# yifita/iso-points

Hardware: AMD Instinct MI355X
Metric: Mpoints/s full iso-point cycle (project+resample+splat), 1M pts (higher is better)
Workload: dtype f32-class (split-fp16 operands, 2^-22: hidden-layer products from two fp16 parts per f32 operand under exact power-of-two scales, 3 fp16-MFMA passes, f32 accumulate; everything else f32)

## Files before the change

### include/isopoints.h

```cpp
#ifndef ISOPOINTS_H_
#define ISOPOINTS_H_

#include <stdint.h>

#ifdef __cplusplus
extern "C" {
#endif

#define ISO_OK 0
#define ISO_ERR_INVALID (-1)
#define ISO_ERR_UNSUPPORTED (-2)
#define ISO_ERR_LAUNCH (-3)
#define ISO_ERR_WORKSPACE (-4)

const char* iso_version(void);
const char* iso_last_error(void);


int iso_project_sphere(const float* pts_in, float* pts_out, float* normals_out,
                       uint8_t* mask_out, int64_t n, float cx, float cy,
                       float cz, float radius, int max_iters, float tol,
                       void* stream);

typedef struct iso_follow {
  void* grid_ws; int64_t grid_n_max;
  const float* views; int n_views; float znear; float zfar; int backface_culling;
  int32_t* mask_out; void* front_ws; int64_t front_ws_bytes;
  int64_t* first_idx_out; int64_t* num_pts_out; int32_t* view_total_out;
} iso_follow;

int iso_project_sphere_follow(const float* pts_in, float* pts_out, float* normals_out,
                              uint8_t* mask_out, int64_t n, float cx, float cy,
                              float cz, float radius, int max_iters, float tol,
                              const iso_follow* follow_host, void* stream);

int64_t iso_siren_raw_floats(int hidden, int n_hidden);
int64_t iso_siren_packed_floats(int hidden, int n_hidden);
int iso_siren_pack_weights(const float* raw, float* packed, int hidden,
                           int n_hidden, void* stream);
int iso_siren_set_gemm_mode(int mode);
int iso_siren_get_gemm_mode(void);
int iso_siren_set_tail_from(int first_tail_iteration);
int iso_siren_set_drawn_tiles(int on);
int iso_idr_set_drawn_tiles(int on);
int iso_siren_set_step_form(int form);
int iso_siren_get_step_form(void);
int iso_siren_step_form_used(int hidden, int n_hidden, int coded);
int iso_siren_step_kernel(int hidden, int n_hidden, int value_only, int coded);
int iso_siren_step_launches(int hidden, int n_hidden, int max_iters);
int64_t iso_project_siren_workspace_bytes(int64_t n, int hidden, int n_hidden);
int64_t iso_project_siren_counts_offset(int64_t n, int hidden, int n_hidden);
int iso_project_siren(const float* pts_in, float* pts_out, float* normals_out,
                      uint8_t* mask_out, int64_t n, const float* packed,
                      int hidden, int n_hidden, float omega_first,
                      float omega_hidden, int max_iters, float tol,
                      void* workspace, int64_t workspace_bytes, void* stream);
int iso_siren_sdf_grad(const float* pts, float* sdf_out, float* grad_out,
                       int64_t n, const float* packed, int hidden,
                       int n_hidden, float omega_first, float omega_hidden,
                       void* workspace, int64_t workspace_bytes, void* stream);

int iso_siren_fold_codes(const float* w0c, const float* b0, const float* codes, float* table, int hidden,
                         int padded_hidden, int c_dim, int64_t n_codes, void* stream);
int iso_project_siren_coded(const float* pts_in, float* pts_out, float* normals_out,
                            uint8_t* mask_out, int64_t n, const float* packed,
                            int hidden, int n_hidden, float omega_first,
                            float omega_hidden, int max_iters, float tol,
                            void* workspace, int64_t workspace_bytes, void* stream,
                            const float* code_bias, const int32_t* code_of, int64_t n_codes);
int iso_siren_sdf_grad_coded(const float* pts, float* sdf_out, float* grad_out,
                             int64_t n, const float* packed, int hidden,
                             int n_hidden, float omega_first, float omega_hidden,
                             void* workspace, int64_t workspace_bytes, void* stream,
                             const float* code_bias, const int32_t* code_of, int64_t n_codes);

int iso_idr_set_gemm_mode(int mode);
int iso_idr_get_gemm_mode(void);
int iso_idr_step_form(int hidden, int n_layers, int skip_layer, int n_freq, int value_only);
int64_t iso_idr_raw_floats(int hidden, int n_layers, int skip_layer, int n_freq);
int64_t iso_idr_packed_floats(int hidden, int n_layers);
int iso_idr_pack_weights(const float* raw, float* packed, int hidden, int n_layers,
                         int skip_layer, int n_freq, void* stream);
int64_t iso_project_idr_workspace_bytes(int64_t n, int hidden, int n_layers);
int iso_project_idr(const float* pts_in, float* pts_out, float* normals_out, uint8_t* mask_out,
                    int64_t n, const float* packed, int hidden, int n_layers, int skip_layer,
                    int n_freq, float beta, int max_iters, float tol, void* workspace,
                    int64_t workspace_bytes, void* stream);
int iso_idr_sdf_grad(const float* pts, float* sdf_out, float* grad_out, int64_t n,
                     const float* packed, int hidden, int n_layers, int skip_layer, int n_freq,
                     float beta, void* workspace, int64_t workspace_bytes, void* stream);

int iso_trace_sphere(const float* ray0, const float* dirs, float* pts_out, float* sdf_out,
// ... 428 lines not shown
```

### iso_points_amd/_lib.py

```python
import ctypes
import os

import torch

_HERE = os.path.dirname(os.path.abspath(__file__))
LIB_PATH = os.path.join(_HERE, "libisopoints_hip.so")
if os.environ.get("ISO_DEV_LIB"):
    LIB_PATH = os.path.abspath(os.environ["ISO_DEV_LIB"])

_c = ctypes
_P = _c.c_void_p
_I = _c.c_int
_L = _c.c_int64
_F = _c.c_float

SIGNATURES = {
    "iso_version": (_c.c_char_p, []),
    "iso_last_error": (_c.c_char_p, []),
    "iso_project_sphere": (_I, [_P, _P, _P, _P, _L, _F, _F, _F, _F, _I, _F, _P]),
    "iso_project_sphere_follow": (_I, [_P, _P, _P, _P, _L, _F, _F, _F, _F, _I, _F, _P, _P]),
    "iso_siren_raw_floats": (_L, [_I, _I]),
    "iso_siren_packed_floats": (_L, [_I, _I]),
    "iso_siren_set_gemm_mode": (_I, [_I]),
    "iso_siren_get_gemm_mode": (_I, []),
    "iso_siren_set_tail_from": (_I, [_I]),
    "iso_siren_set_drawn_tiles": (_I, [_I]),
    "iso_idr_set_drawn_tiles": (_I, [_I]),
    "iso_siren_set_step_form": (_I, [_I]),
    "iso_siren_get_step_form": (_I, []),
    "iso_siren_step_form_used": (_I, [_I, _I, _I]),
    "iso_siren_step_kernel": (_I, [_I, _I, _I, _I]),
    "iso_siren_step_launches": (_I, [_I, _I, _I]),
    "iso_siren_pack_weights": (_I, [_P, _P, _I, _I, _P]),
    "iso_project_siren_workspace_bytes": (_L, [_L, _I, _I]),
    "iso_project_siren_counts_offset": (_L, [_L, _I, _I]),
    "iso_project_siren": (_I, [_P, _P, _P, _P, _L, _P, _I, _I, _F, _F, _I, _F, _P, _L, _P]),
    "iso_siren_sdf_grad": (_I, [_P, _P, _P, _L, _P, _I, _I, _F, _F, _P, _L, _P]),
    "iso_idr_set_gemm_mode": (_I, [_I]),
    "iso_idr_get_gemm_mode": (_I, []),
    "iso_idr_step_form": (_I, [_I, _I, _I, _I, _I]),
    "iso_idr_raw_floats": (_L, [_I, _I, _I, _I]),
    "iso_idr_packed_floats": (_L, [_I, _I]),
    "iso_idr_pack_weights": (_I, [_P, _P, _I, _I, _I, _I, _P]),
    "iso_project_idr_workspace_bytes": (_L, [_L, _I, _I]),
    "iso_project_idr": (_I, [_P, _P, _P, _P, _L, _P, _I, _I, _I, _I, _F, _I, _F, _P, _L, _P]),
    "iso_idr_sdf_grad": (_I, [_P, _P, _P, _L, _P, _I, _I, _I, _I, _F, _P, _L, _P]),
    "iso_trace_sphere": (_I, [_P, _P, _P, _P, _P, _L, _F, _F, _F, _F, _F, _F, _I, _F, _P]),
    "iso_trace_siren": (_I, [_P, _P, _P, _P, _P, _L, _P, _I, _I, _F, _F, _F, _F, _I, _F, _P, _L, _P]),
    "iso_siren_fold_codes": (_I, [_P, _P, _P, _P, _I, _I, _I, _L, _P]),
    "iso_project_siren_coded": (_I, [_P, _P, _P, _P, _L, _P, _I, _I, _F, _F, _I, _F, _P, _L, _P, _P, _P, _L]),
    "iso_siren_sdf_grad_coded": (_I, [_P, _P, _P, _L, _P, _I, _I, _F, _F, _P, _L, _P, _P, _P, _L]),
    "iso_trace_siren_coded": (_I, [_P, _P, _P, _P, _P, _L, _P, _I, _I, _F, _F, _F, _F, _I, _F, _P, _L, _P, _P, _P, _L]),
    "iso_trace_idr": (_I, [_P, _P, _P, _P, _P, _L, _P, _I, _I, _I, _I, _F, _F, _F, _I, _F, _P, _L, _P]),
    "iso_ray_nearest_point_workspace_bytes": (_L, [_L]),
    "iso_ray_nearest_point": (_I, [_P, _L, _F, _F, _F, _P, _L, _P, _P, _P, _P, _L, _P]),
    "iso_raymarch_settle": (_I, [_P, _P, _L, _P, _P, _P, _P, _F, _I, _I, _P, _P, _P, _P]),
    "iso_raymarch_overshoot": (_I, [_P, _P, _L, _P, _P, _P, _P, _I, _I, _F, _P, _P, _P, _P]),
    "iso_raymarch_secant": (_I, [_P, _P, _L, _P, _P, _P, _P, _P, _P, _P, _P]),
    "iso_image_sample": (_I, [_P, _I, _I, _I, _I, _P, _L, _I, _P, _P]),
    "iso_ear_candidates": (_I, [_P, _P, _P, _P, _L, _I, _F, _P, _P, _P]),
    "iso_points_bbox": (_I, [_P, _P, _I, _L, _P, _P]),
    "iso_frnn_make_grid": (_I, [_P, _P, _P, _I, _L, _I, _P, _P]),
    "iso_frnn_make_grid_density": (_I, [_P, _P, _P, _I, _L, _I, _F, _P, _P]),
    "iso_frnn_insert_points": (_I, [_P, _P, _P, _P, _P, _P, _I, _L, _L, _I, _P]),
    "iso_prefix_sum_workspace_bytes": (_L, [_L, _I]),
    "iso_prefix_sum": (_I, [_P, _P, _L, _I, _L, _P, _L, _P]),
    "iso_frnn_scan_cells": (_I, [_P, _P, _P, _I, _L, _I, _P, _L, _P]),
    "iso_frnn_counting_sort": (_I, [_P, _P, _P, _P, _P, _P, _P, _I, _L, _L, _I, _P]),
    "iso_frnn_query_workspace_bytes": (_L, [_I, _L, _L]),
    "iso_frnn_query": (_I, [_P, _P, _P, _P, _P, _P, _P, _P, _P, _I, _P, _P, _P, _I, _L, _L, _L, _P, _L, _P]),
    "iso_frnn_query_others": (_I, [_P, _P, _P, _P, _P, _P, _P, _I, _P, _P, _P, _I, _L, _L, _P, _L, _P]),
    "iso_frnn_gather": (_I, [_P, _P, _P, _I, _L, _L, _I, _I, _P]),
    "iso_repulse": (_I, [_P, _P, _P, _L, _P, _L, _L, _I, _P, _P]),
    "iso_upsample_candidates": (_I, [_P, _P, _L, _I, _P, _P, _P]),
    "iso_farthest_point_sampling_work_floats": (_L, [_I, _L]),
    "iso_farthest_point_sampling": (_I, [_P, _P, _P, _P, _I, _L, _L, _P, _P, _P]),
    "iso_farthest_point_sampling_form": (_I, [_L, _I]),
    "iso_pca_frames_work_bytes": (_L, [_I]),
    "iso_pca_frames": (_I, [_P, _P, _P, _I, _L, _I, _I, _P, _P, _P, _P]),
    "iso_pca_frames_backward_work_bytes": (_L, [_I, _L, _I]),
    "iso_pca_frames_backward": (_I, [_P, _P, _P, _I, _L, _I, _I, _P, _P, _P, _P, _P, _L, _P, _P]),
    "iso_splat_view_flags": (_I, [_P, _P, _P, _P, _L, _I, _F, _F, _I, _P]),
    "iso_compact_rows": (_I, [_P, _P, _P, _P, _L, _L, _I, _P]),
    "iso_splat_vrk_h": (_I, [_P, _P, _P, _P, _P, _I, _L, _P]),
    "iso_splat_setup": (_I, [_P, _P, _P, _P, _P, _P, _P, _I, _L, _I, _F, _F, _P, _P, _P, _P, _P, _P]),
    "iso_splat_vrk_h_global_work_bytes": (_L, [_I]),
# ... 149 lines not shown
```

### iso_points_amd/csrc/siren.hip

```cpp
#include <stdlib.h>
#include <string.h>
#include "siren_common.h"

namespace {

bool siren_shape_ok(int H, int L) {
  return (H == 64 || H == 128 || H == 256) && L >= 0 && L <= 8;
}

int g_gemm_mode = -1;
int gemm_mode() {
  if (g_gemm_mode < 0) {
    const char* e = getenv("ISO_SIREN_GEMM");
    g_gemm_mode = (e && (!strcmp(e, "f32") || !strcmp(e, "0"))) ? 0 : 1;
  }
  return g_gemm_mode;
}

int g_step_form = 1;

int siren_form(int hidden, int n_hidden, bool value_only, bool coded) {
  if (!siren_shape_ok(hidden, n_hidden)) return -1;
  const int NT = hidden / 16;
  if (gemm_mode() == 0 || !siren_x3_supported(hidden, n_hidden)) return 100 + NT;
  if (value_only) return 200 + NT;
  if (hidden == 256 && g_step_form == 1 && (n_hidden == 2 || n_hidden == 3) && !coded) return 500 + NT;
  return (hidden == 128 ? 300 : 400) + NT;
}

int siren_launch_form(int form, const SirenCodedArgs& a, int64_t n, hipStream_t s) {
  switch (form / 100) {
    case 1: return siren_f32_launch(a, 16 * (form % 100), n, s);
    case 2: case 3: case 4: case 5: return siren_x3_launch(form, a, n, s);
    default: return -1;
  }
}

bool form_splits(int form) { return form / 100 >= 4; }

int g_tail_from = -1;
int siren_tail_first(int form, int max_iters) {
  if (!form_splits(form) || g_tail_from == 0) return max_iters + 1;
  if (g_tail_from > 0) return g_tail_from;
  return max_iters >= 6 ? 4 : 2;
}

int g_dyn_tiles = -1;

int64_t stash_floats_any(int H, int L) {
  int64_t a = siren_f32_stash_floats(H, L);
  int64_t b = siren_x3_supported(H, L) ? siren_x3_stash_floats(H, L) : 0;
  return a > b ? a : b;
}

constexpr int kTileCtrInts = 128;
struct SirenCarve {
  int64_t idxA, idxB, tail, tail_counts, counts, tile_ctr, end, tail_cap;
};
SirenCarve siren_carve(int64_t n, int H, int L) {
  if (n < 0) n = 0;
  const int64_t blocks = siren_x3_tail_blocks(), tiles = (n + 31) / 32;
  SirenCarve c;
  c.tail_cap = ((tiles + blocks - 1) / blocks + 1) * 32;
  c.idxA = stash_floats_any(H, L) * 4;
  c.idxB = c.idxA + n * 4;
  c.tail = c.idxB + n * 4;
  c.tail_counts = c.tail + blocks * 2 * c.tail_cap * 4;
  c.counts = c.tail_counts + blocks * 2 * 4;
  c.tile_ctr = c.counts + 64 * 4;
  c.end = c.tile_ctr + kTileCtrInts * 4 + 64;
  return c;
}

__global__ void k_siren_zero(int32_t* c, int n, int32_t* tc, int m) {
  const int i = blockIdx.x * blockDim.x + threadIdx.x;
  if (i < n) c[i] = 0;
  if (i < m) tc[i] = 0;
}

struct SirenTrace { const float* dirs; float alpha, bound; };
struct SirenCodes { const float* bias; const int32_t* of; };

int siren_codes_ok(const char* who, const float* code_bias, const int32_t* code_of, int64_t n_codes) {
  ISO_REQUIRE(code_bias && n_codes >= 1 && (code_of || n_codes == 1), ISO_ERR_INVALID,
              "%s: needs a bias table of n_codes >= 1 rows (and code_of when n_codes > 1)", who);
  return ISO_OK;
}

int siren_run(const char* who, bool ptrs_ok, const float* pts_in, float* pts_out, float* normals_out, uint8_t* mask_out,
              float* sdf_out, float* grad_out, int64_t n, const float* packed, int hidden, int n_hidden, float omega_first,
              float omega_hidden, int max_iters, float tol, void* workspace, int64_t workspace_bytes, void* stream,
              bool eval_only, const SirenTrace* trace, SirenCodes codes) {
  ISO_REQUIRE(siren_shape_ok(hidden, n_hidden), ISO_ERR_UNSUPPORTED,
// ... 56 lines not shown
  ISO_CHECK_LAUNCH(who);
  return ISO_OK;
}

}

extern "C" int64_t iso_siren_raw_floats(int hidden, int n_hidden) {
  int64_t H = hidden;
  return H * 3 + H + (int64_t)n_hidden * (H * H + H) + H + 1;
}

extern "C" int64_t iso_siren_packed_floats(int hidden, int n_hidden) {
  return siren_packed_total(hidden, n_hidden);
}

extern "C" int iso_siren_set_gemm_mode(int mode) {
  ISO_REQUIRE(mode == 0 || mode == 1, ISO_ERR_INVALID, "iso_siren_set_gemm_mode: mode must be 0 (f32 MFMA) or 1 (split fp16)");
  g_gemm_mode = mode;
  return ISO_OK;
}
extern "C" int iso_siren_get_gemm_mode(void) { return gemm_mode(); }

extern "C" int iso_siren_set_step_form(int form) {
  ISO_REQUIRE(form == 0 || form == 1, ISO_ERR_INVALID, "iso_siren_set_step_form: 0 (eight waves, global stash) or 1 (four waves, stash on chip)");
  g_step_form = form;
  return ISO_OK;
}
extern "C" int iso_siren_get_step_form(void) { return g_step_form; }

extern "C" int iso_siren_set_drawn_tiles(int on) {
  ISO_REQUIRE(on >= -1 && on <= 1, ISO_ERR_INVALID, "iso_siren_set_drawn_tiles: -1 (default), 0 or 1");
  g_dyn_tiles = on;
  return ISO_OK;
}

extern "C" int iso_siren_set_tail_from(int first_tail_iteration) {
  ISO_REQUIRE(first_tail_iteration >= -1, ISO_ERR_INVALID, "iso_siren_set_tail_from: -1 (default), 0 (never) or an iteration >= 1");
  g_tail_from = first_tail_iteration;
  return ISO_OK;
}

extern "C" int iso_siren_step_kernel(int hidden, int n_hidden, int value_only, int coded) {
  return siren_form(hidden, n_hidden, value_only != 0, coded != 0);
}
extern "C" int iso_siren_step_form_used(int hidden, int n_hidden, int coded) {
  return siren_form(hidden, n_hidden, false, coded != 0) / 100 == 5 ? 1 : 0;
}
extern "C" int iso_siren_step_launches(int hidden, int n_hidden, int max_iters) {
  if (max_iters < 0) return 0;
  const int from = siren_tail_first(siren_form(hidden, n_hidden, false, false), max_iters);
  return from <= max_iters && from > 0 ? from + 1 : max_iters + 1;
}

extern "C" int iso_siren_pack_weights(const float* raw, float* packed, int hidden,
                                      int n_hidden, void* stream) {
  ISO_REQUIRE(siren_shape_ok(hidden, n_hidden), ISO_ERR_UNSUPPORTED,
              "iso_siren_pack_weights: hidden must be 64/128/256 and 0<=n_hidden<=8 (got %d, %d)",
              hidden, n_hidden);
  ISO_REQUIRE(raw && packed, ISO_ERR_INVALID, "iso_siren_pack_weights: null pointer");
  siren_f32_pack(raw, packed, hidden, n_hidden, (hipStream_t)stream);
  if (hidden % 32 == 0) siren_x3_pack(raw, packed, hidden, n_hidden, (hipStream_t)stream);
  ISO_CHECK_LAUNCH("iso_siren_pack_weights");
  return ISO_OK;
}

extern "C" int64_t iso_project_siren_workspace_bytes(int64_t n, int hidden, int n_hidden) {
  return siren_carve(n, hidden, n_hidden).end;
}
extern "C" int64_t iso_project_siren_counts_offset(int64_t n, int hidden, int n_hidden) {
  return siren_carve(n, hidden, n_hidden).counts;
}

__global__ void k_siren_fold_codes(const float* __restrict__ w0c, const float* __restrict__ b0,
                                   const float* __restrict__ codes, float* __restrict__ table, int H, int Hp, int C,
                                   int64_t U) {
  const int64_t total = U * Hp;
  for (int64_t o = (int64_t)blockIdx.x * blockDim.x + threadIdx.x; o < total; o += (int64_t)gridDim.x * blockDim.x) {
    const int64_t u = o / Hp;
    const int f = (int)(o - u * Hp);
    float v = 0.f;
    if (f < H) {
      double acc = (double)b0[f];
      const float* wr = w0c + (int64_t)f * C;
      const float* cu = codes + u * C;
      for (int k = 0; k < C; ++k) acc = fma((double)wr[k], (double)cu[k], acc);
      v = (float)acc;
    }
    table[o] = v;
  }
}

extern "C" int iso_siren_fold_codes(const float* w0c, const float* b0, const float* codes, float* table, int hidden,
                                    int padded_hidden, int c_dim, int64_t n_codes, void* stream) {
  ISO_REQUIRE(hidden >= 1 && padded_hidden >= hidden && c_dim >= 1 && n_codes >= 0, ISO_ERR_INVALID,
              "iso_siren_fold_codes: bad sizes (hidden %d, padded %d, c_dim %d, codes %lld)", hidden, padded_hidden,
              c_dim, (long long)n_codes);
  if (n_codes == 0) return ISO_OK;
  ISO_REQUIRE(w0c && b0 && codes && table, ISO_ERR_INVALID, "iso_siren_fold_codes: null pointer");
  const int64_t total = n_codes * padded_hidden;
  hipLaunchKernelGGL(k_siren_fold_codes, dim3(iso_stream_grid(total, 256)), dim3(256), 0, (hipStream_t)stream, w0c, b0,
                     codes, table, hidden, padded_hidden, c_dim, n_codes);
  ISO_CHECK_LAUNCH("iso_siren_fold_codes");
  return ISO_OK;
}

static int project_siren(const char* who, const float* pts_in, float* pts_out, float* normals_out, uint8_t* mask_out,
                         int64_t n, const float* packed, int hidden, int n_hidden, float omega_first, float omega_hidden,
                         int max_iters, float tol, void* workspace, int64_t workspace_bytes, void* stream, SirenCodes codes) {
  return siren_run(who, pts_in && pts_out && normals_out && mask_out, pts_in, pts_out, normals_out, mask_out, nullptr,
                   nullptr, n, packed, hidden, n_hidden, omega_first, omega_hidden, max_iters, tol, workspace,
                   workspace_bytes, stream, false, nullptr, codes);
}

extern "C" int iso_project_siren(const float* pts_in, float* pts_out, float* normals_out,
// ... 77 lines not shown
```

### iso_points_amd/csrc/siren_common.h

```cpp
#pragma once
#include "iso_common.h"

struct SirenArgs {
  float* pts;
  float* normals;
  uint8_t* mask;
  float* sdf_out;
  float* grad_out;
  const int32_t* idx_in;
  const int32_t* count_in;
  int32_t* idx_out;
  int32_t* count_out;
  const float* packed;
  float* stash;
  int64_t n;
  int L;
  float w0, wh, tol;
  int do_move;
  int eval_only;
  const float* dirs = nullptr;
  float alpha = 1.f, bound = 0.f, tol_valid = 0.f;
  int fwd_only = 0;
  int64_t cnt_lo = -1, cnt_hi = INT64_MAX;
  int small_tiles = 0;
  int split = 0;
  int big_blocks = 0;
  int32_t* tail_lists = nullptr;
  int32_t* tail_counts = nullptr;
  int32_t* iter_counts = nullptr;
  int tail_cap = 0, it_first = 0, it_last = 0;
  int32_t* tile_ctr = nullptr;
  int draw_first = 0;
  int ps_guard = 0;
};

struct SirenCodedArgs : SirenArgs {
  const float* code_bias = nullptr;
  const int32_t* code_of = nullptr;
};
template <bool CODED> struct SirenArgsOf { using type = SirenArgs; };
template <> struct SirenArgsOf<true> { using type = SirenCodedArgs; };

__host__ __device__ inline int64_t siren_split_point(int64_t count) {
  const int64_t big = 256 * 96, small = 256 * 32;
  const int64_t full = count / big * big, rem = count - full;
  if (rem == 0) return count;
  return (rem + small - 1) / small <= 2 ? full : count;
}

__host__ __device__ inline int64_t off_w0(int H) { (void)H; return 0; }
__host__ __device__ inline int64_t off_wl(int H) { return 4 * (int64_t)H; }
__host__ __device__ inline int64_t off_bl(int H) { return 5 * (int64_t)H; }
__host__ __device__ inline int64_t off_hidden(int H, int l) {
  return 5 * (int64_t)H + 4 + (int64_t)l * ((int64_t)H + 2 * (int64_t)H * H);
}

__host__ __device__ inline int x3_feat(int s, int kappa) {
  return 32 * (s >> 1) + 16 * (s & 1) + 8 * ((kappa & 7) >> 2) + 4 * (kappa >> 3) + (kappa & 3);
}
__host__ __device__ inline int64_t x3_base(int H, int L) { return off_hidden(H, L); }
__host__ __device__ inline int64_t x3_off_w0(int H, int L) { return x3_base(H, L); }
__host__ __device__ inline int64_t x3_off_wl(int H, int L) { return x3_base(H, L) + 4 * (int64_t)H; }
__host__ __device__ inline int64_t x3_off_layer(int H, int L, int l) {
  return x3_base(H, L) + 5 * (int64_t)H + (int64_t)l * (int64_t)H;
}
constexpr int kX16Header = 24;
__host__ __device__ inline int64_t x16_base(int H, int L) { return x3_off_layer(H, L, L); }
__host__ __device__ inline int64_t x16_off_layer(int H, int L, int l) { return x16_base(H, L) + kX16Header + (int64_t)l * H * H; }
__host__ __device__ inline int64_t x16_off_bw(int H, int L, int l) { return x16_off_layer(H, L, L) + (int64_t)l * H * H; }
__host__ __device__ inline int64_t siren_packed_total(int H, int L) { return x16_off_bw(H, L, L); }

void siren_f32_pack(const float* raw, float* packed, int H, int L, hipStream_t s);
int64_t siren_f32_stash_floats(int H, int L);
int siren_f32_launch(const SirenCodedArgs& a, int H, int64_t n, hipStream_t s);
bool siren_x3_supported(int H, int L);
int64_t siren_x3_stash_floats(int H, int L);
void siren_x3_pack(const float* raw, float* packed, int H, int L, hipStream_t s);
int siren_x3_launch(int form, const SirenCodedArgs& a, int64_t n_upper, hipStream_t s);
int siren_x3_tail_blocks();
int siren_x3_launch_tail(const SirenCodedArgs& a, int H, hipStream_t s);
constexpr int64_t kPsMinList = 3 * 256 * 128;
__host__ __device__ inline bool siren_ps_takes(int64_t count, int L, const float* hdr , float wh) {
  if (count < kPsMinList) return false;
  float r = 0.f;
  for (int l = 0; l < L; ++l) r = hdr[17 + l] > r ? hdr[17 + l] : r;
  return (wh * r) * 1.01f < 1.0e4f;
}
```

### iso_points_amd/csrc/siren_f32.hip

```cpp
#include "siren_common.h"
#include "iso_newton.h"
#include "mlp_common.h"

namespace {

__global__ void k_siren_pack(const float* __restrict__ raw, float* __restrict__ packed,
                             int H, int L) {
  const int64_t total = off_hidden(H, L);
  const int64_t HH = (int64_t)H * H;
  const int NT = H / 16;
  for (int64_t o = (int64_t)blockIdx.x * blockDim.x + threadIdx.x; o < total;
       o += (int64_t)gridDim.x * blockDim.x) {
    float v = 0.f;
    if (o < off_wl(H)) {
      int64_t k = o;
      int c = (int)(k & 3);
      int e = (int)((k >> 2) % (H / 4));
      int g = (int)((k >> 2) / (H / 4));
      int f = 16 * (e >> 2) + 4 * g + (e & 3);
      v = (c < 3) ? raw[f * 3 + c] : raw[(int64_t)H * 3 + f];
    } else if (o < off_bl(H)) {
      int64_t k = o - off_wl(H);
      int e = (int)(k % (H / 4));
      int g = (int)(k / (H / 4));
      int f = 16 * (e >> 2) + 4 * g + (e & 3);
      const int64_t raw_wl = (int64_t)H * 4 + (int64_t)L * (HH + H);
      v = raw[raw_wl + f];
    } else if (o < off_hidden(H, 0)) {
      const int64_t raw_wl = (int64_t)H * 4 + (int64_t)L * (HH + H);
      v = (o == off_bl(H)) ? raw[raw_wl + H] : 0.f;
    } else {
      int64_t k = o - off_hidden(H, 0);
      const int64_t per = H + 2 * HH;
      int l = (int)(k / per);
      int64_t w = k % per;
      const float* Wl = raw + (int64_t)H * 4 + (int64_t)l * (HH + H);
      const float* bl = Wl + HH;
      if (w < H) {
        v = bl[w];
      } else {
        w -= H;
        bool bwd = w >= HH;
        if (bwd) w -= HH;
        int i = (int)(w & 3);
        int lane = (int)((w >> 2) & 63);
        int t = (int)((w >> 8) % NT);
        int q = (int)((w >> 8) / NT);
        int a = 16 * t + (lane & 15);
        int b = 16 * q + 4 * (lane >> 4) + i;
        v = bwd ? Wl[(int64_t)b * H + a]
                : Wl[(int64_t)a * H + b];
      }
    }
    packed[o] = v;
  }
}

#define ISO_GEMM_FWD(img, bias) gemm_pass<NT, true>(img, bias, hL, wbuf, acc, lane, g)
#define ISO_GEMM_BWD(img) gemm_pass<NT, false>(img, nullptr, hL, wbuf, acc, lane, g)

template <int NT, bool CODED>
__global__ __launch_bounds__(256, 2) void k_siren_step(typename SirenArgsOf<CODED>::type a) {
  constexpr int H = NT * 16;
  extern __shared__ __attribute__((aligned(16))) float smem[];
  const int tid = threadIdx.x;
  const int wave = tid >> 6, lane = tid & 63;
  const int g = lane >> 4, j = lane & 15;
  float* hL = smem + wave * (NT * 256);
  float* wbuf = smem + 4 * NT * 256;
  const float* W0img = a.packed + off_w0(H);
  const float* WLimg = a.packed + off_wl(H);
  const float bL = a.packed[off_bl(H)];
  float* stash = a.stash + ((int64_t)blockIdx.x * 4 + wave) * (int64_t)(a.L + 1) * NT * 256;

  const int64_t count = a.count_in ? (int64_t)(*a.count_in) : a.n;
  const int64_t n_tiles = (count + 63) / 64;
  for (int64_t tile = blockIdx.x; tile < n_tiles; tile += gridDim.x) {
    const int64_t slot = tile * 64 + wave * 16 + j;
    const bool valid = slot < count;
    int64_t idx = -1;
    float px = 0.f, py = 0.f, pz = 0.f;
    int row = 0;
    if (valid) {
      idx = a.idx_in ? (int64_t)a.idx_in[slot] : slot;
      px = a.pts[idx * 3]; py = a.pts[idx * 3 + 1]; pz = a.pts[idx * 3 + 2];
      if constexpr (CODED) row = a.code_of ? a.code_of[idx] : 0;
    }
    const f32x4* cb = nullptr;
    if constexpr (CODED) cb = reinterpret_cast<const f32x4*>(a.code_bias + (int64_t)row * H) + g;
    (void)cb;
    float f = 0.f;
    const bool top0 = (a.L == 0);
    for (int e4 = 0; e4 < NT; ++e4) {
      f32x4 h4, s4;
      f32x4 b4 = {0.f, 0.f, 0.f, 0.f};
      if constexpr (CODED) b4 = cb[4 * e4];
#pragma unroll
      for (int i = 0; i < 4; ++i) {
        const f32x4 w = reinterpret_cast<const f32x4*>(W0img)[g * (H / 4) + e4 * 4 + i];
        float z;
        if constexpr (CODED) z = ((w.x * px + w.y * py) + w.z * pz) + b4[i];
        else z = ((w.x * px + w.y * py) + w.z * pz) + w.w;
        float s, c;
        iso_sincos(a.w0 * z, s, c);
        h4[i] = s;
        s4[i] = a.w0 * c;
      }
      if (top0) {
// ... 122 lines not shown
```

### iso_points_amd/csrc/siren_x3.hip

```cpp
#include <stdlib.h>
#include <type_traits>
#include "siren_common.h"
#include "iso_newton.h"
#include "mlp_common.h"

#include "mfma_split.h"

constexpr int kAD = 3;

namespace {

__device__ __forceinline__ void x3_sin_wcos8(float w_in, float w, const float (&z)[8], float (&s)[8], float (&c)[8]) {
  iso_sin_wcos8(w_in, w, z, s, c);
}


__global__ void k_siren_pack_x3(const float* __restrict__ raw, float* __restrict__ packed, int H, int L) {
  const int64_t base = x3_base(H, L), total = x16_base(H, L);
  const int64_t HH = (int64_t)H * H;
  const float* b0 = raw + (int64_t)H * 3;
  const float* WL = raw + (int64_t)H * 4 + (int64_t)L * (HH + H);
  for (int64_t o = base + (int64_t)blockIdx.x * blockDim.x + threadIdx.x; o < total;
       o += (int64_t)gridDim.x * blockDim.x) {
    const int64_t rel = o - base;
    auto feat_of = [](int64_t ko) { return x3_feat((int)(ko >> 4), 8 * (int)((ko >> 3) & 1) + (int)(ko & 7)); };
    if (rel < 4 * (int64_t)H) {
      const int f = feat_of(rel >> 2), c = (int)(rel & 3);
      packed[o] = (c < 3) ? raw[f * 3 + c] : b0[f];
    } else if (rel < 5 * (int64_t)H) {
      packed[o] = WL[feat_of(rel - 4 * (int64_t)H)];
    } else {
      const int64_t r2 = rel - 5 * (int64_t)H;
      const int l = (int)(r2 / H);
      const float* Wl = raw + (int64_t)H * 4 + (int64_t)l * (HH + H);
      packed[o] = Wl[HH + feat_of(r2 % H)];
    }
  }
}

__global__ void k_siren_wscale(const float* __restrict__ raw, float* __restrict__ packed, int H, int L) {
  __shared__ float s_m[256];
  const int l = blockIdx.x;
  const int64_t HH = (int64_t)H * H;
  const float* Wl = raw + (int64_t)H * 4 + (int64_t)l * (HH + H);
  float m = 0.f, cs = 0.f;
  for (int f = threadIdx.x; f < H; f += 256) {
    float t = 0.f;
#pragma unroll 32
    for (int k = 0; k < H; ++k) {
      const float a = fabsf(Wl[(int64_t)k * H + f]);
      m = (a == a && a > m) ? a : m;
      t += a;
    }
    cs = fmaxf(cs, t);
  }
  s_m[threadIdx.x] = m;
  __syncthreads();
  for (int o = 128; o > 0; o >>= 1) {
    if ((int)threadIdx.x < o) s_m[threadIdx.x] = fmaxf(s_m[threadIdx.x], s_m[threadIdx.x + o]);
    __syncthreads();
  }
  if (threadIdx.x == 0) {
    float mx = s_m[0];
    int e = 0;
    float sc = 1.0f;
    if (mx > 0.f && mx < 3.0e38f) {
      (void)frexpf(mx, &e);
      int k = 10 - e;
      k = k > 100 ? 100 : (k < -100 ? -100 : k);
      sc = ldexpf(1.0f, k);
    }
    packed[x16_base(H, L) + l] = sc;
  }
  __syncthreads();
  s_m[threadIdx.x] = cs;
  __syncthreads();
  for (int o = 128; o > 0; o >>= 1) {
    if ((int)threadIdx.x < o) s_m[threadIdx.x] = fmaxf(s_m[threadIdx.x], s_m[threadIdx.x + o]);
    __syncthreads();
  }
  if (threadIdx.x == 0) packed[x16_base(H, L) + 8 + l] = s_m[0];
  if (l == 0) {
    __syncthreads();
    const float* WLh = raw + (int64_t)H * 4 + (int64_t)L * (HH + H);
    float mh = 0.f;
    for (int f = threadIdx.x; f < H; f += 256) mh = fmaxf(mh, fabsf(WLh[f]));
    s_m[threadIdx.x] = mh;
    __syncthreads();
    for (int o = 128; o > 0; o >>= 1) {
      if ((int)threadIdx.x < o) s_m[threadIdx.x] = fmaxf(s_m[threadIdx.x], s_m[threadIdx.x + o]);
      __syncthreads();
    }
    if (threadIdx.x == 0) packed[x16_base(H, L) + 16] = s_m[0];
  }
}

__global__ void k_siren_pack_f16(const float* __restrict__ raw, float* __restrict__ packed, int H, int L) {
  const int64_t HH = (int64_t)H * H;
  const int NTO = H / 32;
  const int64_t total = 2 * (int64_t)L * HH;
  for (int64_t o = (int64_t)blockIdx.x * blockDim.x + threadIdx.x; o < total; o += (int64_t)gridDim.x * blockDim.x) {
    const bool bwd = o >= (int64_t)L * HH;
    const int l = (int)((o / HH) % L);
    const int64_t q = o % HH;
    const float* Wl = raw + (int64_t)H * 4 + (int64_t)l * (HH + H);
    const float sc = packed[x16_base(H, L) + l];
    const int d = (int)(q & 3), lane = (int)((q >> 2) & 63);
    const int64_t blk = q >> 8;
    const int part = (int)(blk & 1);
    const int To = (int)((blk >> 1) % NTO), s = (int)(blk / (2 * NTO));
    const int fo = 32 * To + (lane & 31);
    f32x2 v;
#pragma unroll
    for (int u = 0; u < 2; ++u) {
      const int fi = x3_feat(s, 8 * (lane >> 5) + 2 * d + u);
      v[u] = (bwd ? Wl[(int64_t)fi * H + fo] : Wl[(int64_t)fo * H + fi]) * sc;
    }
    const f16x2 h = __builtin_convertvector(v, f16x2);
    const f16x2 lo = __builtin_convertvector(v - __builtin_convertvector(h, f32x2), f16x2);
    reinterpret_cast<unsigned*>(packed + x16_off_layer(H, L, 0))[o] =
        part == 0 ? __builtin_bit_cast(unsigned, h) : __builtin_bit_cast(unsigned, lo);
  }
}

template <int H, int NW, int NB, int RP = 1>
struct X3Shape {
  static constexpr int NS = H / 16;
  static constexpr int NTO = H / 32;
  static constexpr int TW = NTO / NW;
  static constexpr int SL = 2 * TW;
  static constexpr int NG = SL * NB;
  static constexpr int P = 32 * NB;
  static constexpr size_t kActBytes = (size_t)NS * NB * kAP * 1024;
  static constexpr size_t kRedBytes = RP > 1 ? (size_t)2 * P * NW * 4 : (size_t)NW * P * 16;
  static constexpr size_t kPtsBytes = (size_t)P * 16;
  static constexpr int kLdsGroupsFit = (int)((163840 - (kActBytes + kRedBytes + kPtsBytes)) / ((size_t)NW * 2048));
  static constexpr int LG = kLdsGroupsFit < NG ? kLdsGroupsFit : NG;
  static constexpr size_t kLds = kActBytes + kRedBytes + kPtsBytes + (size_t)NW * LG * 2048;
  static constexpr int64_t kStashPerWg(int L) { return (int64_t)NW * (L > 1 ? L : 1) * NG * 512; }
  static_assert(NTO % NW == 0 && TW >= 1, "features must split evenly over the waves");
  static_assert(RP == 1 || (size_t)NW * LG * 2048 >= (size_t)NW * RP * P * 16, "the final reduction fits the LDS stash");
};

template <int H>
__device__ __forceinline__ void x3_code_bias8(const float* table, int row, int s, int h, float (&b)[8]) {
  const f32x4* t = reinterpret_cast<const f32x4*>(table + (int64_t)row * H + 16 * s + 4 * h);
  const f32x4 lo = t[0], hi = t[2];
#pragma unroll
  for (int e = 0; e < 4; ++e) { b[e] = lo[e]; b[4 + e] = hi[e]; }
}

template <int H, int NW, int NB, bool FWD, bool CODED, int LT = 0>
__device__ __forceinline__ void x3_step_body(const typename SirenArgsOf<CODED>::type& a, const int bid, const int nblk,
                                             const int sid) {
  constexpr bool RS = LT > 0;
  constexpr int RP = RS ? (H / 32) / NW : 1;
  static_assert(!RS || !FWD, "the on-chip form is a gradient kernel");
  using S = X3Shape<H, NW, NB, RP>;
  constexpr int NS = S::NS, NTO = S::NTO, TW = S::TW, SL = S::SL, NG = S::NG, P = S::P;
  extern __shared__ __attribute__((aligned(16))) unsigned char smem_raw[];
  u32x4* act = reinterpret_cast<u32x4*>(smem_raw);
  f32x4* red = reinterpret_cast<f32x4*>(smem_raw + S::kActBytes);
  f32x4* ptl = reinterpret_cast<f32x4*>(smem_raw + S::kActBytes + S::kRedBytes);
  constexpr int LG = S::LG;
  const int tid = threadIdx.x;
  const int w = __builtin_amdgcn_readfirstlane(tid >> 6);
  const int lane = tid & 63, h = lane >> 5, j = lane & 31;
  u32x4* own = act + (size_t)(SL * w) * NB * kAP * 64 + lane;
  u32x4* park = own + (size_t)(kAP - 2) * NG * 64;
  constexpr bool IL = (NW == 8) || RS;
  const int L = RS ? LT : a.L;
  const float* X = a.packed + x3_base(H, L);
  const f32x4* W0u = reinterpret_cast<const f32x4*>(X) + SL * w * 16;
  const float* WLu = X + 4 * H + SL * w * 16;
  const int h8 = h * 8;
// ... 529 lines not shown
  return 0;
}

template <int H, int NW, int NB, int MINB, bool CODED, int LT = 0>
int launch_x3_both(typename SirenArgsOf<CODED>::type a, int64_t n_upper, hipStream_t s) {
  constexpr int RP = LT > 0 ? (H / 32) / NW : 1;
  using SB = X3Shape<H, NW, NB, RP>;
  using SS = X3Shape<H, NW, 1, RP>;
  static_assert(LT == 0 || NW == kOcNW, "the on-chip form: four waves");
  constexpr size_t lds = SB::kLds > SS::kLds ? SB::kLds : SS::kLds;
  static_assert(lds <= 163840, "LDS of a gfx950 CU");
  void (*kern)(typename SirenArgsOf<CODED>::type);
  if constexpr (LT > 0) kern = &k_siren_step_x3_both_oc<H, NB, MINB, CODED, LT>;
  else kern = &k_siren_step_x3_both<H, NW, NB, MINB, CODED>;
  static bool attr_done = false;
  if (!attr_done) {
    (void)hipFuncSetAttribute(reinterpret_cast<const void*>(kern), hipFuncAttributeMaxDynamicSharedMemorySize, (int)lds);
    attr_done = true;
  }
  const int64_t cap = 256 * MINB;
  const int64_t tb = (n_upper + SB::P - 1) / SB::P, ts = (n_upper + SS::P - 1) / SS::P;
  a.big_blocks = (int)(tb < cap ? (tb < 1 ? 1 : tb) : cap);
  a.split = 3;
  const int small_blocks = (int)(ts < cap ? (ts < 1 ? 1 : ts) : cap);
  hipLaunchKernelGGL(kern, dim3(a.big_blocks + small_blocks), dim3(64 * NW), lds, s, a);
  return 0;
}

}

constexpr int kNW256 = 8;
constexpr int kMinB256 = 1;
constexpr int kNB256 = 3;
constexpr int kMinB128 = 1;
bool siren_x3_supported(int H, int L) { return (H == 256 || H == 128) && L >= 1 && L <= 8; }

int64_t siren_x3_stash_floats(int H, int L) {
  if (H == 256) {
    return 256 * kMinB256 * (X3Shape<256, kNW256, kNB256>::kStashPerWg(L) + X3Shape<256, kNW256, 1>::kStashPerWg(L));
  }
  if (H == 128) return 256 * kMinB128 * X3Shape<128, 4, 3>::kStashPerWg(L);
  return 0;
}

void siren_x3_pack(const float* raw, float* packed, int H, int L, hipStream_t s) {
  const int64_t words = x16_base(H, L) - x3_base(H, L);
  hipLaunchKernelGGL(k_siren_pack_x3, dim3(iso_stream_grid(words, 256)), dim3(256), 0, s, raw, packed, H, L);
  if (L > 0) {
    hipLaunchKernelGGL(k_siren_wscale, dim3(L), dim3(256), 0, s, raw, packed, H, L);
    hipLaunchKernelGGL(k_siren_pack_f16, dim3(iso_stream_grid(2 * (int64_t)L * H * H, 256)), dim3(256), 0, s, raw, packed, H, L);
  }
}

int siren_x3_tail_blocks() { return 256 * kMinB256; }

template <bool CODED>
static int launch_tail(const typename SirenArgsOf<CODED>::type& a, hipStream_t s) {
  using SS = X3Shape<256, kNW256, 1>;
  static bool attr_done = false;
  if (!attr_done) {
    (void)hipFuncSetAttribute(reinterpret_cast<const void*>(&k_siren_tail_x3<256, kNW256, kMinB256, CODED>),
                              hipFuncAttributeMaxDynamicSharedMemorySize, (int)SS::kLds);
    attr_done = true;
  }
  hipLaunchKernelGGL((k_siren_tail_x3<256, kNW256, kMinB256, CODED>), dim3(siren_x3_tail_blocks()), dim3(64 * kNW256), SS::kLds, s, a);
  return 0;
}

int siren_x3_launch_tail(const SirenCodedArgs& a, int H, hipStream_t s) {
  if (H != 256) return -1;
  return a.code_bias ? launch_tail<true>(a, s) : launch_tail<false>(a, s);
}

template <bool CODED>
static int launch_form(int form, const typename SirenArgsOf<CODED>::type& a, int64_t n_upper, hipStream_t s) {
  switch (form) {
    case 208: return launch_x3<128, 4, 3, kMinB128, true, CODED>(a, n_upper, s);
    case 216: return launch_x3<256, kNW256, kNB256, kMinB256, true, CODED>(a, n_upper, s);
    case 308: return launch_x3<128, 4, 3, kMinB128, false, CODED>(a, n_upper, s);
    case 416: return launch_x3_both<256, kNW256, kNB256, kMinB256, CODED>(a, n_upper, s);
    case 516:
      if constexpr (!CODED) {
        if (a.L == 2) return launch_x3_both<256, kOcNW, kNB256, kMinB256, false, 2>(a, n_upper, s);
        if (a.L == 3) return launch_x3_both<256, kOcNW, kNB256, kMinB256, false, 3>(a, n_upper, s);
      }
      return -1;
    default: return -1;
  }
}

int siren_x3_launch(int form, const SirenCodedArgs& a, int64_t n_upper, hipStream_t s) {
  return a.code_bias ? launch_form<true>(form, a, n_upper, s) : launch_form<false>(form, a, n_upper, s);
}
```

Before: 88.78.

## Fuse SIREN weight packing into a single multi-section kernel launch

```diff
diff --git a/include/isopoints.h b/include/isopoints.h
--- a/include/isopoints.h
+++ b/include/isopoints.h
@@ -38,6 +38,7 @@
 int64_t iso_siren_packed_floats(int hidden, int n_hidden);
 int iso_siren_pack_weights(const float* raw, float* packed, int hidden,
                            int n_hidden, void* stream);
+int iso_siren_set_pack_form(int form);
 int iso_siren_set_gemm_mode(int mode);
 int iso_siren_get_gemm_mode(void);
 int iso_siren_set_tail_from(int first_tail_iteration);
diff --git a/iso_points_amd/_lib.py b/iso_points_amd/_lib.py
--- a/iso_points_amd/_lib.py
+++ b/iso_points_amd/_lib.py
@@ -32,6 +32,7 @@
     "iso_siren_step_kernel": (_I, [_I, _I, _I, _I]),
     "iso_siren_step_launches": (_I, [_I, _I, _I]),
     "iso_siren_pack_weights": (_I, [_P, _P, _I, _I, _P]),
+    "iso_siren_set_pack_form": (_I, [_I]),
     "iso_project_siren_workspace_bytes": (_L, [_L, _I, _I]),
     "iso_project_siren_counts_offset": (_L, [_L, _I, _I]),
     "iso_project_siren": (_I, [_P, _P, _P, _P, _L, _P, _I, _I, _F, _F, _I, _F, _P, _L, _P]),
diff --git a/iso_points_amd/csrc/siren.hip b/iso_points_amd/csrc/siren.hip
--- a/iso_points_amd/csrc/siren.hip
+++ b/iso_points_amd/csrc/siren.hip
@@ -39,6 +39,7 @@
 bool form_splits(int form) { return form / 100 >= 4; }
 
 int g_tail_from = -1;
+int g_pack_form = 1;
 int siren_tail_first(int form, int max_iters) {
   if (!form_splits(form) || g_tail_from == 0) return max_iters + 1;
   if (g_tail_from > 0) return g_tail_from;
@@ -201,14 +202,24 @@
   return from <= max_iters && from > 0 ? from + 1 : max_iters + 1;
 }
 
+extern "C" int iso_siren_set_pack_form(int form) {
+  ISO_REQUIRE(form == 0 || form == 1, ISO_ERR_INVALID, "iso_siren_set_pack_form: 0 (a launch per section) or 1 (one launch)");
+  g_pack_form = form;
+  return ISO_OK;
+}
+
 extern "C" int iso_siren_pack_weights(const float* raw, float* packed, int hidden,
                                       int n_hidden, void* stream) {
   ISO_REQUIRE(siren_shape_ok(hidden, n_hidden), ISO_ERR_UNSUPPORTED,
               "iso_siren_pack_weights: hidden must be 64/128/256 and 0<=n_hidden<=8 (got %d, %d)",
               hidden, n_hidden);
   ISO_REQUIRE(raw && packed, ISO_ERR_INVALID, "iso_siren_pack_weights: null pointer");
-  siren_f32_pack(raw, packed, hidden, n_hidden, (hipStream_t)stream);
-  if (hidden % 32 == 0) siren_x3_pack(raw, packed, hidden, n_hidden, (hipStream_t)stream);
+  if (g_pack_form != 0 && hidden % 32 == 0) {
+    siren_pack_all(raw, packed, hidden, n_hidden, (hipStream_t)stream);
+  } else {
+    siren_f32_pack(raw, packed, hidden, n_hidden, (hipStream_t)stream);
+    if (hidden % 32 == 0) siren_x3_pack(raw, packed, hidden, n_hidden, (hipStream_t)stream);
+  }
   ISO_CHECK_LAUNCH("iso_siren_pack_weights");
   return ISO_OK;
 }
diff --git a/iso_points_amd/csrc/siren_common.h b/iso_points_amd/csrc/siren_common.h
--- a/iso_points_amd/csrc/siren_common.h
+++ b/iso_points_amd/csrc/siren_common.h
@@ -76,6 +76,7 @@
 bool siren_x3_supported(int H, int L);
 int64_t siren_x3_stash_floats(int H, int L);
 void siren_x3_pack(const float* raw, float* packed, int H, int L, hipStream_t s);
+void siren_pack_all(const float* raw, float* packed, int H, int L, hipStream_t s);
 int siren_x3_launch(int form, const SirenCodedArgs& a, int64_t n_upper, hipStream_t s);
 int siren_x3_tail_blocks();
 int siren_x3_launch_tail(const SirenCodedArgs& a, int H, hipStream_t s);
diff --git a/iso_points_amd/csrc/siren_f32.hip b/iso_points_amd/csrc/siren_f32.hip
--- a/iso_points_amd/csrc/siren_f32.hip
+++ b/iso_points_amd/csrc/siren_f32.hip
@@ -1,59 +1,16 @@
 #include "siren_common.h"
 #include "iso_newton.h"
 #include "mlp_common.h"
+#include "siren_pack.h"
 
 namespace {
 
 __global__ void k_siren_pack(const float* __restrict__ raw, float* __restrict__ packed,
                              int H, int L) {
   const int64_t total = off_hidden(H, L);
-  const int64_t HH = (int64_t)H * H;
-  const int NT = H / 16;
   for (int64_t o = (int64_t)blockIdx.x * blockDim.x + threadIdx.x; o < total;
-       o += (int64_t)gridDim.x * blockDim.x) {
-    float v = 0.f;
-    if (o < off_wl(H)) {
-      int64_t k = o;
-      int c = (int)(k & 3);
-      int e = (int)((k >> 2) % (H / 4));
-      int g = (int)((k >> 2) / (H / 4));
-      int f = 16 * (e >> 2) + 4 * g + (e & 3);
-      v = (c < 3) ? raw[f * 3 + c] : raw[(int64_t)H * 3 + f];
-    } else if (o < off_bl(H)) {
-      int64_t k = o - off_wl(H);
-      int e = (int)(k % (H / 4));
-      int g = (int)(k / (H / 4));
-      int f = 16 * (e >> 2) + 4 * g + (e & 3);
-      const int64_t raw_wl = (int64_t)H * 4 + (int64_t)L * (HH + H);
-      v = raw[raw_wl + f];
-    } else if (o < off_hidden(H, 0)) {
-      const int64_t raw_wl = (int64_t)H * 4 + (int64_t)L * (HH + H);
-      v = (o == off_bl(H)) ? raw[raw_wl + H] : 0.f;
-    } else {
-      int64_t k = o - off_hidden(H, 0);
-      const int64_t per = H + 2 * HH;
-      int l = (int)(k / per);
-      int64_t w = k % per;
-      const float* Wl = raw + (int64_t)H * 4 + (int64_t)l * (HH + H);
-      const float* bl = Wl + HH;
-      if (w < H) {
-        v = bl[w];
-      } else {
-        w -= H;
-        bool bwd = w >= HH;
-        if (bwd) w -= HH;
-        int i = (int)(w & 3);
-        int lane = (int)((w >> 2) & 63);
-        int t = (int)((w >> 8) % NT);
-        int q = (int)((w >> 8) / NT);
-        int a = 16 * t + (lane & 15);
-        int b = 16 * q + 4 * (lane >> 4) + i;
-        v = bwd ? Wl[(int64_t)b * H + a]
-                : Wl[(int64_t)a * H + b];
-      }
-    }
-    packed[o] = v;
-  }
+       o += (int64_t)gridDim.x * blockDim.x)
+    packed[o] = siren_pack_f32_word(raw, H, L, o);
 }
 
 #define ISO_GEMM_FWD(img, bias) gemm_pass<NT, true>(img, bias, hL, wbuf, acc, lane, g)
diff --git a/iso_points_amd/csrc/siren_pack.h b/iso_points_amd/csrc/siren_pack.h
--- /dev/null
+++ b/iso_points_amd/csrc/siren_pack.h
@@ -0,0 +1,167 @@
+#pragma once
+#include <math.h>
+#include "siren_common.h"
+#include "mfma_split.h"
+
+#pragma clang fp contract(off)
+
+namespace {
+
+__device__ __forceinline__ float siren_pack_f32_word(const float* __restrict__ raw, int H, int L, int64_t o) {
+  const int64_t HH = (int64_t)H * H;
+  const int NT = H / 16;
+  float v = 0.f;
+  if (o < off_wl(H)) {
+    int64_t k = o;
+    int c = (int)(k & 3);
+    int e = (int)((k >> 2) % (H / 4));
+    int g = (int)((k >> 2) / (H / 4));
+    int f = 16 * (e >> 2) + 4 * g + (e & 3);
+    v = (c < 3) ? raw[f * 3 + c] : raw[(int64_t)H * 3 + f];
+  } else if (o < off_bl(H)) {
+    int64_t k = o - off_wl(H);
+    int e = (int)(k % (H / 4));
+    int g = (int)(k / (H / 4));
+    int f = 16 * (e >> 2) + 4 * g + (e & 3);
+    const int64_t raw_wl = (int64_t)H * 4 + (int64_t)L * (HH + H);
+    v = raw[raw_wl + f];
+  } else if (o < off_hidden(H, 0)) {
+    const int64_t raw_wl = (int64_t)H * 4 + (int64_t)L * (HH + H);
+    v = (o == off_bl(H)) ? raw[raw_wl + H] : 0.f;
+  } else {
+    int64_t k = o - off_hidden(H, 0);
+    const int64_t per = H + 2 * HH;
+    int l = (int)(k / per);
+    int64_t w = k % per;
+    const float* Wl = raw + (int64_t)H * 4 + (int64_t)l * (HH + H);
+    const float* bl = Wl + HH;
+    if (w < H) {
+      v = bl[w];
+    } else {
+      w -= H;
+      bool bwd = w >= HH;
+      if (bwd) w -= HH;
+      int i = (int)(w & 3);
+      int lane = (int)((w >> 2) & 63);
+      int t = (int)((w >> 8) % NT);
+      int q = (int)((w >> 8) / NT);
+      int a = 16 * t + (lane & 15);
+      int b = 16 * q + 4 * (lane >> 4) + i;
+      v = bwd ? Wl[(int64_t)b * H + a]
+              : Wl[(int64_t)a * H + b];
+    }
+  }
+  return v;
+}
+
+__device__ __forceinline__ float siren_pack_x3_word(const float* __restrict__ raw, int H, int L, int64_t rel) {
+  const int64_t HH = (int64_t)H * H;
+  const float* b0 = raw + (int64_t)H * 3;
+  const float* WL = raw + (int64_t)H * 4 + (int64_t)L * (HH + H);
+  auto feat_of = [](int64_t ko) { return x3_feat((int)(ko >> 4), 8 * (int)((ko >> 3) & 1) + (int)(ko & 7)); };
+  if (rel < 4 * (int64_t)H) {
+    const int f = feat_of(rel >> 2), c = (int)(rel & 3);
+    return (c < 3) ? raw[f * 3 + c] : b0[f];
+  }
+  if (rel < 5 * (int64_t)H) return WL[feat_of(rel - 4 * (int64_t)H)];
+  const int64_t r2 = rel - 5 * (int64_t)H;
+  const int l = (int)(r2 / H);
+  const float* Wl = raw + (int64_t)H * 4 + (int64_t)l * (HH + H);
+  return Wl[HH + feat_of(r2 % H)];
+}
+
+__device__ __forceinline__ float siren_block_max256(float v, float* s_m) {
+  s_m[threadIdx.x] = v;
+  __syncthreads();
+  for (int o = 128; o > 0; o >>= 1) {
+    if ((int)threadIdx.x < o) s_m[threadIdx.x] = fmaxf(s_m[threadIdx.x], s_m[threadIdx.x + o]);
+    __syncthreads();
+  }
+  const float m = s_m[0];
+  __syncthreads();
+  return m;
+}
+
+__device__ __forceinline__ float siren_wscale_of(float mx) {
+  int e = 0;
+  float sc = 1.0f;
+  if (mx > 0.f && mx < 3.0e38f) {
+    (void)frexpf(mx, &e);
+    int k = 10 - e;
+    k = k > 100 ? 100 : (k < -100 ? -100 : k);
+    sc = ldexpf(1.0f, k);
+  }
+  return sc;
+}
+
+__device__ __forceinline__ void siren_wscale_layer(const float* __restrict__ raw, float* __restrict__ packed, int H, int L,
+                                                   int l, float* s_m) {
+  const int64_t HH = (int64_t)H * H;
+  const float* Wl = raw + (int64_t)H * 4 + (int64_t)l * (HH + H);
+  float m = 0.f, cs = 0.f;
+  for (int f = threadIdx.x; f < H; f += 256) {
+    float t = 0.f;
+#pragma unroll 32
+    for (int k = 0; k < H; ++k) {
+      const float a = fabsf(Wl[(int64_t)k * H + f]);
+      m = (a == a && a > m) ? a : m;
+      t += a;
+    }
+    cs = fmaxf(cs, t);
+  }
+  const float mx = siren_block_max256(m, s_m);
+  if (threadIdx.x == 0) packed[x16_base(H, L) + l] = siren_wscale_of(mx);
+  const float c = siren_block_max256(cs, s_m);
+  if (threadIdx.x == 0) packed[x16_base(H, L) + 8 + l] = c;
+  if (l == 0) {
+    const float* WLh = raw + (int64_t)H * 4 + (int64_t)L * (HH + H);
+    float mh = 0.f;
+    for (int f = threadIdx.x; f < H; f += 256) mh = fmaxf(mh, fabsf(WLh[f]));
+    const float hm = siren_block_max256(mh, s_m);
+    if (threadIdx.x == 0) packed[x16_base(H, L) + 16] = hm;
+  }
+}
+
+__device__ __forceinline__ float siren_wscale_only(const float* __restrict__ raw, int H, int l, float* s_m) {
+  const int64_t HH = (int64_t)H * H;
+  const float* Wl = raw + (int64_t)H * 4 + (int64_t)l * (HH + H);
+  float m = 0.f;
+  auto take = [&](float w) { const float a = fabsf(w); m = (a == a && a > m) ? a : m; };
+  if ((reinterpret_cast<uintptr_t>(Wl) & 15) == 0) {
+    const float4* W4 = reinterpret_cast<const float4*>(Wl);
+#pragma unroll 16
+    for (int64_t i = threadIdx.x; i < HH / 4; i += 256) {
+      const float4 w = W4[i];
+      take(w.x); take(w.y); take(w.z); take(w.w);
+    }
+  } else {
+#pragma unroll 32
+    for (int64_t i = threadIdx.x; i < HH; i += 256) take(Wl[i]);
+  }
+  return siren_wscale_of(siren_block_max256(m, s_m));
+}
+
+__device__ __forceinline__ unsigned siren_pack_f16_word(const float* __restrict__ raw, int H, int L, int64_t o, float sc) {
+  const int64_t HH = (int64_t)H * H;
+  const int NTO = H / 32;
+  const bool bwd = o >= (int64_t)L * HH;
+  const int l = (int)((o / HH) % L);
+  const int64_t q = o % HH;
+  const float* Wl = raw + (int64_t)H * 4 + (int64_t)l * (HH + H);
+  const int d = (int)(q & 3), lane = (int)((q >> 2) & 63);
+  const int64_t blk = q >> 8;
+  const int part = (int)(blk & 1);
+  const int To = (int)((blk >> 1) % NTO), s = (int)(blk / (2 * NTO));
+  const int fo = 32 * To + (lane & 31);
+  f32x2 v;
+#pragma unroll
+  for (int u = 0; u < 2; ++u) {
+    const int fi = x3_feat(s, 8 * (lane >> 5) + 2 * d + u);
+    v[u] = (bwd ? Wl[(int64_t)fi * H + fo] : Wl[(int64_t)fo * H + fi]) * sc;
+  }
+  const f16x2 h = __builtin_convertvector(v, f16x2);
+  const f16x2 lo = __builtin_convertvector(v - __builtin_convertvector(h, f32x2), f16x2);
+  return part == 0 ? __builtin_bit_cast(unsigned, h) : __builtin_bit_cast(unsigned, lo);
+}
+
+}
diff --git a/iso_points_amd/csrc/siren_x3.hip b/iso_points_amd/csrc/siren_x3.hip
--- a/iso_points_amd/csrc/siren_x3.hip
+++ b/iso_points_amd/csrc/siren_x3.hip
@@ -5,6 +5,7 @@
 #include "mlp_common.h"
 
 #include "mfma_split.h"
+#include "siren_pack.h"
 
 constexpr int kAD = 3;
 
@@ -17,110 +18,55 @@
 
 __global__ void k_siren_pack_x3(const float* __restrict__ raw, float* __restrict__ packed, int H, int L) {
   const int64_t base = x3_base(H, L), total = x16_base(H, L);
-  const int64_t HH = (int64_t)H * H;
-  const float* b0 = raw + (int64_t)H * 3;
-  const float* WL = raw + (int64_t)H * 4 + (int64_t)L * (HH + H);
   for (int64_t o = base + (int64_t)blockIdx.x * blockDim.x + threadIdx.x; o < total;
-       o += (int64_t)gridDim.x * blockDim.x) {
-    const int64_t rel = o - base;
-    auto feat_of = [](int64_t ko) { return x3_feat((int)(ko >> 4), 8 * (int)((ko >> 3) & 1) + (int)(ko & 7)); };
-    if (rel < 4 * (int64_t)H) {
-      const int f = feat_of(rel >> 2), c = (int)(rel & 3);
-      packed[o] = (c < 3) ? raw[f * 3 + c] : b0[f];
-    } else if (rel < 5 * (int64_t)H) {
-      packed[o] = WL[feat_of(rel - 4 * (int64_t)H)];
-    } else {
-      const int64_t r2 = rel - 5 * (int64_t)H;
-      const int l = (int)(r2 / H);
-      const float* Wl = raw + (int64_t)H * 4 + (int64_t)l * (HH + H);
-      packed[o] = Wl[HH + feat_of(r2 % H)];
-    }
-  }
+       o += (int64_t)gridDim.x * blockDim.x)
+    packed[o] = siren_pack_x3_word(raw, H, L, o - base);
 }
 
 __global__ void k_siren_wscale(const float* __restrict__ raw, float* __restrict__ packed, int H, int L) {
   __shared__ float s_m[256];
-  const int l = blockIdx.x;
-  const int64_t HH = (int64_t)H * H;
-  const float* Wl = raw + (int64_t)H * 4 + (int64_t)l * (HH + H);
-  float m = 0.f, cs = 0.f;
-  for (int f = threadIdx.x; f < H; f += 256) {
-    float t = 0.f;
-#pragma unroll 32
-    for (int k = 0; k < H; ++k) {
-      const float a = fabsf(Wl[(int64_t)k * H + f]);
-      m = (a == a && a > m) ? a : m;
-      t += a;
-    }
-    cs = fmaxf(cs, t);
-  }
-  s_m[threadIdx.x] = m;
-  __syncthreads();
-  for (int o = 128; o > 0; o >>= 1) {
-    if ((int)threadIdx.x < o) s_m[threadIdx.x] = fmaxf(s_m[threadIdx.x], s_m[threadIdx.x + o]);
-    __syncthreads();
-  }
-  if (threadIdx.x == 0) {
-    float mx = s_m[0];
-    int e = 0;
-    float sc = 1.0f;
-    if (mx > 0.f && mx < 3.0e38f) {
-      (void)frexpf(mx, &e);
-      int k = 10 - e;
-      k = k > 100 ? 100 : (k < -100 ? -100 : k);
-      sc = ldexpf(1.0f, k);
-    }
-    packed[x16_base(H, L) + l] = sc;
-  }
-  __syncthreads();
-  s_m[threadIdx.x] = cs;
-  __syncthreads();
-  for (int o = 128; o > 0; o >>= 1) {
-    if ((int)threadIdx.x < o) s_m[threadIdx.x] = fmaxf(s_m[threadIdx.x], s_m[threadIdx.x + o]);
-    __syncthreads();
-  }
-  if (threadIdx.x == 0) packed[x16_base(H, L) + 8 + l] = s_m[0];
-  if (l == 0) {
-    __syncthreads();
-    const float* WLh = raw + (int64_t)H * 4 + (int64_t)L * (HH + H);
-    float mh = 0.f;
-    for (int f = threadIdx.x; f < H; f += 256) mh = fmaxf(mh, fabsf(WLh[f]));
-    s_m[threadIdx.x] = mh;
-    __syncthreads();
-    for (int o = 128; o > 0; o >>= 1) {
-      if ((int)threadIdx.x < o) s_m[threadIdx.x] = fmaxf(s_m[threadIdx.x], s_m[threadIdx.x + o]);
-      __syncthreads();
-    }
-    if (threadIdx.x == 0) packed[x16_base(H, L) + 16] = s_m[0];
-  }
+  siren_wscale_layer(raw, packed, H, L, blockIdx.x, s_m);
 }
 
 __global__ void k_siren_pack_f16(const float* __restrict__ raw, float* __restrict__ packed, int H, int L) {
   const int64_t HH = (int64_t)H * H;
-  const int NTO = H / 32;
   const int64_t total = 2 * (int64_t)L * HH;
   for (int64_t o = (int64_t)blockIdx.x * blockDim.x + threadIdx.x; o < total; o += (int64_t)gridDim.x * blockDim.x) {
-    const bool bwd = o >= (int64_t)L * HH;
-    const int l = (int)((o / HH) % L);
-    const int64_t q = o % HH;
-    const float* Wl = raw + (int64_t)H * 4 + (int64_t)l * (HH + H);
-    const float sc = packed[x16_base(H, L) + l];
-    const int d = (int)(q & 3), lane = (int)((q >> 2) & 63);
-    const int64_t blk = q >> 8;
-    const int part = (int)(blk & 1);
-    const int To = (int)((blk >> 1) % NTO), s = (int)(blk / (2 * NTO));
-    const int fo = 32 * To + (lane & 31);
-    f32x2 v;
-#pragma unroll
-    for (int u = 0; u < 2; ++u) {
-      const int fi = x3_feat(s, 8 * (lane >> 5) + 2 * d + u);
-      v[u] = (bwd ? Wl[(int64_t)fi * H + fo] : Wl[(int64_t)fo * H + fi]) * sc;
-    }
-    const f16x2 h = __builtin_convertvector(v, f16x2);
-    const f16x2 lo = __builtin_convertvector(v - __builtin_convertvector(h, f32x2), f16x2);
-    reinterpret_cast<unsigned*>(packed + x16_off_layer(H, L, 0))[o] =
-        part == 0 ? __builtin_bit_cast(unsigned, h) : __builtin_bit_cast(unsigned, lo);
-  }
+    const float sc = packed[x16_base(H, L) + (int)((o / HH) % L)];
+    reinterpret_cast<unsigned*>(packed + x16_off_layer(H, L, 0))[o] = siren_pack_f16_word(raw, H, L, o, sc);
+  }
+}
+
+constexpr int kPackSliceWords = 1024;
+__global__ __launch_bounds__(256) void k_siren_pack_all(const float* __restrict__ raw, float* __restrict__ packed, int H,
+                                                        int L, int n_x3, int n_f32) {
+  __shared__ float s_m[256];
+  const int64_t HH = (int64_t)H * H;
+  const int S = (int)(HH / kPackSliceWords);
+  int b = blockIdx.x;
+  if (b < L) { siren_wscale_layer(raw, packed, H, L, b, s_m); return; }
+  b -= L;
+  if (b < L * S) {
+    const int l = b / S, slice = b % S;
+    const float sc = siren_wscale_only(raw, H, l, s_m);
+    unsigned* img = reinterpret_cast<unsigned*>(packed + x16_off_layer(H, L, 0));
+    for (int dir = 0; dir < 2; ++dir) {
+      const int64_t o0 = ((int64_t)dir * L + l) * HH + (int64_t)slice * kPackSliceWords;
+      for (int k = threadIdx.x; k < kPackSliceWords; k += 256) img[o0 + k] = siren_pack_f16_word(raw, H, L, o0 + k, sc);
+    }
+    return;
+  }
+  b -= L * S;
+  if (b < n_x3) {
+    const int64_t words = x16_base(H, L) - x3_base(H, L);
+    for (int64_t rel = (int64_t)b * 256 + threadIdx.x; rel < words; rel += (int64_t)n_x3 * 256)
+      packed[x3_base(H, L) + rel] = siren_pack_x3_word(raw, H, L, rel);
+    return;
+  }
+  b -= n_x3;
+  const int64_t total = off_hidden(H, L);
+  for (int64_t o = (int64_t)b * 256 + threadIdx.x; o < total; o += (int64_t)n_f32 * 256)
+    packed[o] = siren_pack_f32_word(raw, H, L, o);
 }
 
 template <int H, int NW, int NB, int RP = 1>
@@ -756,6 +702,12 @@
   }
 }
 
+void siren_pack_all(const float* raw, float* packed, int H, int L, hipStream_t s) {
+  const int n_x3 = iso_stream_grid(x16_base(H, L) - x3_base(H, L), 256), n_f32 = iso_stream_grid(off_hidden(H, L), 256);
+  const int n_16 = L * (int)((int64_t)H * H / kPackSliceWords);
+  hipLaunchKernelGGL(k_siren_pack_all, dim3(L + n_16 + n_x3 + n_f32), dim3(256), 0, s, raw, packed, H, L, n_x3, n_f32);
+}
+
 int siren_x3_tail_blocks() { return 256 * kMinB256; }
 
 template <bool CODED>
```

New measurement: 88.76 (median of 3 runs). Within noise of the previous version (-0.0%).
